# autonomousvision/LaRa

Hardware: AMD Instinct MI355X
Metric: novel-view frames/sec @512x512 (4-view in, 2DGS fwd+bwd) (higher is better)
Workload: dtype f32 raster + bf16-MFMA/f32-accumulate encoder (+ bf16-autocast coarse decoder MLP, as the reference's bf16-mixed)

## Files before the change

### lara_amd/csrc/abi.hip

```cpp
#include <stdlib.h>
#include <string.h>

#include "common.h"

static thread_local int g_last_hip_error = 0;
void l2d_set_hip_error(hipError_t e) { g_last_hip_error = (int)e; }

#include <atomic>
#include <mutex>
#include <map>
#include <utility>
#include <vector>
namespace {
struct ProfRec { const char *name; hipEvent_t a, b; };
std::atomic<bool> g_prof_on{false};
std::mutex g_prof_mu;
std::vector<ProfRec> g_prof_log;
std::vector<hipEvent_t> g_prof_pool;
hipEvent_t prof_event() {
    if (!g_prof_pool.empty()) { hipEvent_t e = g_prof_pool.back(); g_prof_pool.pop_back(); return e; }
    hipEvent_t e = nullptr;
    (void)hipEventCreate(&e);
    return e;
}
}

L2dProfScope::L2dProfScope(const char *name, hipStream_t stream) : slot(-1), s(stream) {
    if (!g_prof_on.load(std::memory_order_relaxed)) return;
    std::lock_guard<std::mutex> lk(g_prof_mu);
    ProfRec r{name, prof_event(), prof_event()};
    (void)hipEventRecord(r.a, s);
    g_prof_log.push_back(r);
    slot = (int)g_prof_log.size() - 1;
}
L2dProfScope::~L2dProfScope() {
    if (slot < 0) return;
    std::lock_guard<std::mutex> lk(g_prof_mu);
    if (slot < (int)g_prof_log.size()) (void)hipEventRecord(g_prof_log[slot].b, s);
}

namespace {

bool make_view(const lara2dgs_view *view, ViewDev &v) {
    if (!view) return false;
    if (view->P < 0 || view->image_height <= 0 || view->image_width <= 0) return false;
    if (view->sh_degree < 0 || view->sh_degree > 3) return false;
    if (view->capacity < 0 || view->capacity > 0xffffffffll) return false;
    if (!view->bg || !view->viewmatrix || !view->projmatrix || !view->campos) return false;
    v.P = view->P;
    v.deg = view->sh_degree;
    v.M = view->sh_coeffs;
    v.H = view->image_height;
    v.W = view->image_width;
    v.gx = (v.W + TILE - 1) / TILE;
    v.gy = (v.H + TILE - 1) / TILE;
    v.tiles = v.gx * v.gy;
    if (v.gx > 65535 || v.gy > 65535) return false;
    v.scale_modifier = view->scale_modifier;
// ... 396 lines not shown
```

### lara_amd/csrc/encoder_bwd.hip

```cpp
#include <cstdlib>

#include "mfma_gemm.h"
#include "mlp_fused.h"
#include "group_attn.h"
#include "../../include/lara_groupattn.h"

namespace {

struct TnP {
    const unsigned short *A, *B;
    float *part;
    const int *nbr;
    int M, lda, ldb, N, Kc, T, chunk, tiles;
};
constexpr int TN_GROUP_MAX = 6;
struct TnGroup {
    TnP p[TN_GROUP_MAX];
    int first_slot[TN_GROUP_MAX + 1];
    int count;
};

__device__ __forceinline__ bf16x8 pack_lo(const uint32_t *w) {
    union { uint32_t u[4]; bf16x8 v; } r;
#pragma unroll
    for (int d = 0; d < 4; d++) r.u[d] = __builtin_amdgcn_perm(w[2 * d + 1], w[2 * d], 0x05040100u);
    return r.v;
}
__device__ __forceinline__ bf16x8 pack_hi(const uint32_t *w) {
    union { uint32_t u[4]; bf16x8 v; } r;
#pragma unroll
    for (int d = 0; d < 4; d++) r.u[d] = __builtin_amdgcn_perm(w[2 * d + 1], w[2 * d], 0x07060302u);
    return r.v;
}
// ... 581 lines not shown
#pragma unroll
            for (int u = 0; u < 16; u++) v[u] = part[(size_t)(q + 16 * u) * stride + c];
#pragma unroll
            for (int u = 0; u < 8; u++) v[u] += v[u + 8];
#pragma unroll
            for (int u = 0; u < 4; u++) v[u] += v[u + 4];
            s += (v[0] + v[2]) + (v[1] + v[3]);
        }
        for (; q < parts; q += 16) s += part[(size_t)q * stride + c];
    }
    red[sl][lane] = s;
    __syncthreads();
    if (sl == 0 && c < n) {
        float t = red[0][lane];
        for (int k = 1; k < 16; k++) t += red[k][lane];
        g.dst[which][c] += t;
    }
}

__global__ void __launch_bounds__(256)
neighbour_table_kernel(int *__restrict__ nbr, const int M, const int R, const int zero_row, const int row_bytes) {
    const int m = blockIdx.x * 256 + threadIdx.x;
    if (m >= M) return;
    int b, d, h, w;
    token_to_voxel(m, R, b, d, h, w);
    for (int tap = 0; tap < 27; tap++) {
        const int nd = d + tap / 9 - 1, nh = h + (tap / 3) % 3 - 1, nw = w + tap % 3 - 1;
        const bool in = (unsigned)nd < (unsigned)R && (unsigned)nh < (unsigned)R && (unsigned)nw < (unsigned)R;
        nbr[(size_t)tap * M + m] = (in ? voxel_to_token(b, nd, nh, nw, R) : zero_row) * row_bytes;
    }
}

constexpr int LNB_ROWS = 128;
template <bool DY_BF16>
__global__ void __launch_bounds__(256)
ln_bwd_kernel(const void *dy_, const float *__restrict__ x, const float *__restrict__ gamma, const float eps,
              const float *skip, float *dx_out, unsigned short *__restrict__ dx_bf16, float *__restrict__ part,
              const int tokens) {
    const float *dy = (const float *)dy_;
    const unsigned short *dyh = (const unsigned short *)dy_;
    auto load_dy = [&](const size_t tok, const int lane) {
        if (DY_BF16) {
            const ushort4 h = ((const ushort4 *)(dyh + tok * 256))[lane];
            return make_float4(bf2f(h.x), bf2f(h.y), bf2f(h.z), bf2f(h.w));
        }
        return ((const float4 *)(dy + tok * 256))[lane];
    };
    __shared__ float red[4][12][64];
    const int wave = threadIdx.x >> 6, lane = threadIdx.x & 63;
    const float4 g = ((const float4 *)gamma)[lane];
    float pg[4] = {0.f, 0.f, 0.f, 0.f}, pb[4] = {0.f, 0.f, 0.f, 0.f}, po[4] = {0.f, 0.f, 0.f, 0.f};
    const int tok0 = blockIdx.x * LNB_ROWS + wave * (LNB_ROWS / 4);
    const int nrow = min(LNB_ROWS / 4, tokens - tok0);
    const float4 z4 = make_float4(0.f, 0.f, 0.f, 0.f);
    float4 vn = z4, dn = z4, kn = z4;
    if (nrow > 0) {
        vn = ((const float4 *)(x + (size_t)tok0 * 256))[lane];
        dn = load_dy((size_t)tok0, lane);
        if (skip) kn = ((const float4 *)(skip + (size_t)tok0 * 256))[lane];
    }
    for (int i = 0; i < nrow; i++) {
        const int tok = tok0 + i;
        const float4 v = vn, d = dn, k = kn;
        if (i + 1 < nrow) {
            vn = ((const float4 *)(x + (size_t)(tok + 1) * 256))[lane];
            dn = load_dy((size_t)(tok + 1), lane);
            if (skip) kn = ((const float4 *)(skip + (size_t)(tok + 1) * 256))[lane];
        }
        float s = v.x + v.y + v.z + v.w;
#pragma unroll
        for (int o = 32; o > 0; o >>= 1) s += __shfl_xor(s, o, 64);
        const float mean = s * (1.0f / 256.0f);
        const float c0 = v.x - mean, c1 = v.y - mean, c2 = v.z - mean, c3 = v.w - mean;
        float q = c0 * c0 + c1 * c1 + c2 * c2 + c3 * c3;
#pragma unroll
        for (int o = 32; o > 0; o >>= 1) q += __shfl_xor(q, o, 64);
        const float rstd = 1.0f / sqrtf(q * (1.0f / 256.0f) + eps);
        const float h0 = c0 * rstd, h1 = c1 * rstd, h2 = c2 * rstd, h3 = c3 * rstd;
        const float a0 = d.x * g.x, a1 = d.y * g.y, a2 = d.z * g.z, a3 = d.w * g.w;
        float sa = a0 + a1 + a2 + a3, sh = a0 * h0 + a1 * h1 + a2 * h2 + a3 * h3;
#pragma unroll
        for (int o = 32; o > 0; o >>= 1) { sa += __shfl_xor(sa, o, 64); sh += __shfl_xor(sh, o, 64); }
        sa *= (1.0f / 256.0f); sh *= (1.0f / 256.0f);
        const float4 r = make_float4(rstd * (a0 - sa - h0 * sh) + k.x, rstd * (a1 - sa - h1 * sh) + k.y,
                                     rstd * (a2 - sa - h2 * sh) + k.z, rstd * (a3 - sa - h3 * sh) + k.w);
        ((float4 *)(dx_out + (size_t)tok * 256))[lane] = r;
        if (dx_bf16) {
            ushort4 hb;
            hb.x = f2bf(r.x); hb.y = f2bf(r.y); hb.z = f2bf(r.z); hb.w = f2bf(r.w);
            ((ushort4 *)(dx_bf16 + (size_t)tok * 256))[lane] = hb;
        }
        pg[0] += d.x * h0; pg[1] += d.y * h1; pg[2] += d.z * h2; pg[3] += d.w * h3;
        pb[0] += d.x; pb[1] += d.y; pb[2] += d.z; pb[3] += d.w;
        po[0] += r.x; po[1] += r.y; po[2] += r.z; po[3] += r.w;
    }
#pragma unroll
    for (int c = 0; c < 4; c++) { red[wave][c][lane] = pg[c]; red[wave][4 + c][lane] = pb[c]; red[wave][8 + c][lane] = po[c]; }
    __syncthreads();
    if (wave == 0) {
#pragma unroll
        for (int k = 0; k < 12; k++) {
            const float t = (red[0][k][lane] + red[1][k][lane]) + (red[2][k][lane] + red[3][k][lane]);
            part[(size_t)blockIdx.x * 768 + (k >> 2) * 256 + 4 * lane + (k & 3)] = t;
        }
    }
}

__global__ void __launch_bounds__(256)
colsum_bf16_kernel(const unsigned short *__restrict__ src, float *__restrict__ part, const int rows, const int C) {
    const int r0 = blockIdx.x * 64, r1 = min(rows, r0 + 64);
    for (int c2 = threadIdx.x; c2 < C / 2; c2 += 256) {
        float s0 = 0.f, s1 = 0.f;
        for (int rr = r0; rr < r1; rr++) {
            const uint32_t w = *(const uint32_t *)(src + (size_t)rr * C + 2 * c2);
            s0 += __uint_as_float(w << 16);
            s1 += __uint_as_float(w & 0xffff0000u);
        }
        part[(size_t)blockIdx.x * C + 2 * c2] = s0;
        part[(size_t)blockIdx.x * C + 2 * c2 + 1] = s1;
    }
}

__global__ void __launch_bounds__(256)
// ... 100 lines not shown
    if (active) {
#pragma unroll
        for (int d = 0; d < 8; d++) {
            s_kv[gl][j2 * 512 + h2 * 16 + d0 + d] = f2bf(dk[d]);
            s_kv[gl][j2 * 512 + 256 + h2 * 16 + d0 + d] = f2bf(dvv[d]);
        }
    }
    __syncthreads();
    if (active) {
        uint4 *oq = (uint4 *)(dQ + (size_t)g * 8 * 256);
        unsigned short *ok = dKV + ((size_t)g * 4 + (t >> 6)) * lddkv + (t & 63) * 8;
        oq[t] = ((const uint4 *)s_dq[gl])[t]; oq[t + 128] = ((const uint4 *)s_dq[gl])[t + 128];
        *(uint4 *)ok = ((const uint4 *)s_kv[gl])[t]; *(uint4 *)(ok + 2 * (size_t)lddkv) = ((const uint4 *)s_kv[gl])[t + 128];
    }
}

constexpr size_t TN_PART_BYTES = 128ull << 20;

inline int cu_count() {
    static const int cus = [] {
        int dev = 0, v = 0;
        if (hipGetDevice(&dev) != hipSuccess || hipDeviceGetAttribute(&v, hipDeviceAttributeMultiprocessorCount, dev) != hipSuccess) v = 0;
        return v > 0 ? v : 256;
    }();
    return cus;
}

struct TnJob {
    const unsigned short *A; int lda, N;
    const unsigned short *B; int ldb, Kc;
    int M;
    float *dst;
};
int gemm_tn_group(const TnJob *jobs, int count, float *part, hipStream_t s);
inline bool tn_ring_shape(int M, int N, int Kc, int lda, int ldb, const float *dst) {
    return M >= 128 && !(M & 127) && !(N & 255) && !(Kc & 7) && !(lda & 7) && !(ldb & 7) && (size_t)(M + 1) * lda * 2 < (1ull << 32) &&
           (size_t)(M + 1) * ldb * 2 < (1ull << 32) && M < (1 << 24) && ldb < (1 << 23) && (((uintptr_t)dst) & 15) == 0;
}

int gemm_tn(const unsigned short *A, int lda, int N, const unsigned short *B, int ldb, int Kc, int T, const int *nbr,
            int M, float *dst, float *part, hipStream_t s) {
    if (M <= 0 || (nbr && M < 16) || (N & 1) || (Kc & 1) || (T > 1 && (Kc & 127))) return LARA2DGS_E_INVALID;
    if ((size_t)(M + 1) * lda * 2 >= (1ull << 32) || (size_t)(M + 1) * ldb * 2 >= (1ull << 32) || M >= (1 << 24) || ldb >= (1 << 23))
        return LARA2DGS_E_INVALID;
    const size_t out_bytes = (size_t)N * T * Kc * 4;
    const int n = N * T * Kc;
    if (!nbr && T == 1 && tn_ring_shape(M, N, Kc, lda, ldb, dst)) {
        const TnJob j{A, lda, N, B, ldb, Kc, M, dst};
        return gemm_tn_group(&j, 1, part, s);
    }
    if (nbr && N == 256 && Kc == 256 && (M & 127) == 0 && !(lda & 7) && !(ldb & 7) && (((uintptr_t)dst | (uintptr_t)part) & 15) == 0) {
        const int cus = cu_count();
        static const hipError_t attr = hipFuncSetAttribute((const void *)gemm_tn_ring_kernel<true>,
                                                           hipFuncAttributeMaxDynamicSharedMemorySize, TR_RING * TR_STAGE);
        L2D_HIP(attr);
        const int g128 = M / 128;
        int splits = max(1, min(min(cus / T, g128), (int)(TN_PART_BYTES / out_bytes)));
        const int chunk = ((g128 + splits - 1) / splits) * 128;
        splits = (M + chunk - 1) / chunk;
        TnRingGroup g{};
        TnRingP &q = g.p[0];
        q.A = A; q.B = B; q.part = part; q.nbr = nbr; q.M = M; q.lda = lda; q.ldb = ldb; q.T = T; q.ntile = q.ktile = 1; q.Kc = 256;
        q.chunk = chunk; q.splits = splits;
        g.count = 1; g.first_wg[0] = 0; g.first_wg[1] = T * splits;
        L2D_LAUNCH_IN_SCOPE(s, gemm_tn_ring_kernel<true>, dim3(T * splits), dim3(512), TR_RING * TR_STAGE, g);
        L2D_LAUNCH_IN_SCOPE(s, accum_partials4_kernel, dim3((n / 4 + 63) / 64), dim3(256), 0, dst, part, n, splits, (size_t)n);
        return LARA2DGS_OK;
    }
    const int tiles = ((N + 127) / 128) * ((Kc + 127) / 128) * T;
    const int want = 1024;
    int splits = max(1, min(want / tiles, (int)(TN_PART_BYTES / out_bytes)));
    splits = max(8, splits & ~7);
    while (splits > 8 && M / splits < 256) splits -= 8;
    const int chunk = (((M + splits - 1) / splits) + 63) & ~63;
    TnP p{};
    p.A = A; p.B = B; p.part = part; p.nbr = nbr; p.M = M; p.lda = lda; p.ldb = ldb; p.N = N; p.Kc = Kc; p.T = T;
    p.chunk = chunk; p.tiles = tiles;
    if ((size_t)splits * out_bytes > TN_PART_BYTES) return LARA2DGS_E_INVALID;
    const bool staged = !((M & 31) || (N & 7) || (Kc & 7) || (lda & 7) || (ldb & 7));
    if (staged) {
        TnGroup g{};
        g.p[0] = p; g.count = 1; g.first_slot[0] = 0; g.first_slot[1] = tiles * splits / 8;
        if (nbr) L2D_LAUNCH_IN_SCOPE(s, (gemm_bf16_tn_lds_kernel<true>), dim3(tiles * splits), dim3(256), 0, g);
        else L2D_LAUNCH_IN_SCOPE(s, (gemm_bf16_tn_lds_kernel<false>), dim3(tiles * splits), dim3(256), 0, g);
    } else {
        if (nbr) L2D_LAUNCH_IN_SCOPE(s, (gemm_bf16_tn_kernel<true>), dim3(tiles * splits), dim3(256), 0, p);
        else L2D_LAUNCH_IN_SCOPE(s, (gemm_bf16_tn_kernel<false>), dim3(tiles * splits), dim3(256), 0, p);
    }
    if ((n & 3) == 0 && (((uintptr_t)dst | (uintptr_t)part) & 15) == 0 && (n / 4 + 63) / 64 < 128 && splits >= 64)
        L2D_LAUNCH_IN_SCOPE(s, accum_partials4_wide_kernel, dim3((n / 4 + 63) / 64), dim3(1024), 0, dst, part, n, splits, (size_t)n);
    else if ((n & 3) == 0 && (((uintptr_t)dst | (uintptr_t)part) & 15) == 0)
        L2D_LAUNCH_IN_SCOPE(s, accum_partials4_kernel, dim3((n / 4 + 63) / 64), dim3(256), 0, dst, part, n, splits, (size_t)n);
    else
        L2D_LAUNCH_IN_SCOPE(s, accum_partials_kernel, dim3((n + 63) / 64), dim3(256), 0, dst, part, n, splits, (size_t)n);
    return LARA2DGS_OK;
}

int gemm_tn_group(const TnJob *jobs, int count, float *part, hipStream_t s) {
    bool ok = count >= 1 && count <= TN_GROUP_MAX;
    int tiles_all = 0;
    for (int k = 0; k < count && ok; k++) {
        const TnJob &j = jobs[k];
        ok = !((j.M & 31) || (j.N & 7) || (j.Kc & 7) || (j.lda & 7) || (j.ldb & 7)) && ((j.N * j.Kc) & 3) == 0 &&
             (size_t)(j.M + 1) * j.lda * 2 < (1ull << 32) && (size_t)(j.M + 1) * j.ldb * 2 < (1ull << 32) && j.M < (1 << 24) &&
             j.ldb < (1 << 23) && (((uintptr_t)j.dst) & 15) == 0;
        tiles_all += ((j.N + 127) / 128) * ((j.Kc + 127) / 128);
    }
    if (!ok) {
        for (int k = 0; k < count; k++) {
            L2D_TRY(gemm_tn(jobs[k].A, jobs[k].lda, jobs[k].N, jobs[k].B, jobs[k].ldb, jobs[k].Kc, 1, nullptr, jobs[k].M,
                                   jobs[k].dst, part, s));
        }
        return LARA2DGS_OK;
    }
    bool ringable = true;
    long units = 0;
    for (int k = 0; k < count; k++) {
        const TnJob &j = jobs[k];
        ringable = ringable && tn_ring_shape(j.M, j.N, j.Kc, j.lda, j.ldb, j.dst);
        units += (long)(j.N / 256) * ((j.Kc + 255) / 256) * (j.M / 128);
    }
    if (ringable) {
        static const hipError_t attr = hipFuncSetAttribute((const void *)gemm_tn_ring_kernel<false>,
                                                           hipFuncAttributeMaxDynamicSharedMemorySize, TR_RING * TR_STAGE);
        L2D_HIP(attr);
        const int cus = cu_count();
        TnRingGroup g{};
        AccGroup a{};
        g.count = a.count = count;
        for (int cg = (int)max(1l, (units + cus - 1) / cus);; cg++) {
            int wgs = 0, rwg = 0;
            size_t off_f = 0;
            for (int k = 0; k < count; k++) {
                const TnJob &j = jobs[k];
                const int tiles = (j.N / 256) * ((j.Kc + 255) / 256), n = j.N * j.Kc, splits = (j.M / 128 + cg - 1) / cg;
                TnRingP &q = g.p[k];
                q.A = j.A; q.B = j.B; q.part = part + off_f; q.nbr = nullptr; q.M = j.M; q.lda = j.lda; q.ldb = j.ldb; q.T = 1;
                q.ntile = j.N / 256; q.ktile = (j.Kc + 255) / 256; q.Kc = j.Kc; q.chunk = cg * 128; q.splits = splits;
                g.first_wg[k] = wgs;
                wgs += tiles * splits;
                a.dst[k] = j.dst; a.part[k] = part + off_f; a.n[k] = n; a.parts[k] = splits; a.first_wg[k] = rwg;
                rwg += (n / 4 + 63) / 64;
                off_f += (size_t)splits * n;
            }
            g.first_wg[count] = wgs;
            a.first_wg[count] = rwg;
            if (wgs <= cus && off_f * 4 <= TN_PART_BYTES) break;
            if (cg > (1 << 20)) return LARA2DGS_E_INVALID;
        }
        L2D_LAUNCH_IN_SCOPE(s, gemm_tn_ring_kernel<false>, dim3(g.first_wg[count]), dim3(512), TR_RING * TR_STAGE, g);
        L2D_LAUNCH_IN_SCOPE(s, accum_partials4_group_kernel, dim3(a.first_wg[count]), dim3(256), 0, a);
        return LARA2DGS_OK;
    }
    const int want = 1280;
    int base = max(8, (want / tiles_all) & ~7);
    TnGroup g{};
    AccGroup a{};
    g.count = a.count = count;
    size_t off_f = 0;
    for (;;) {
        off_f = 0;
        int slot = 0, wg = 0;
        for (int k = 0; k < count; k++) {
            const TnJob &j = jobs[k];
            int splits = base;
            while (splits > 8 && j.M / splits < 256) splits -= 8;
            const int tiles = ((j.N + 127) / 128) * ((j.Kc + 127) / 128), n = j.N * j.Kc;
            TnP &p = g.p[k];
            p.A = j.A; p.B = j.B; p.part = part + off_f; p.nbr = nullptr; p.M = j.M; p.lda = j.lda; p.ldb = j.ldb; p.N = j.N; p.Kc = j.Kc;
            p.T = 1; p.chunk = (((j.M + splits - 1) / splits) + 63) & ~63; p.tiles = tiles;
            g.first_slot[k] = slot;
            slot += tiles * splits / 8;
            a.dst[k] = j.dst; a.part[k] = part + off_f; a.n[k] = n; a.parts[k] = splits; a.first_wg[k] = wg;
            wg += (n / 4 + 63) / 64;
            off_f += (size_t)splits * n;
        }
        g.first_slot[count] = slot;
        a.first_wg[count] = wg;
        if (off_f * 4 <= TN_PART_BYTES || base == 8) break;
        base -= 8;
    }
    if (off_f * 4 > TN_PART_BYTES) return LARA2DGS_E_INVALID;
    L2D_LAUNCH_IN_SCOPE(s, (gemm_bf16_tn_lds_kernel<false>), dim3(g.first_slot[count] * 8), dim3(256), 0, g);
    L2D_LAUNCH_IN_SCOPE(s, accum_partials4_group_kernel, dim3(a.first_wg[count]), dim3(256), 0, a);
    return LARA2DGS_OK;
}

struct RedList {
    RedGroup g{};
    int wgs = 0;
    bool overflow = false;
    void add(float *dst, const float *part, int n, int parts, int stride) {
        if (!dst) return;
        if (g.count >= RED_GROUP_MAX) { overflow = true; return; }
        const int k = g.count++;
        g.dst[k] = dst; g.part[k] = part; g.n[k] = n; g.parts[k] = parts; g.stride[k] = stride; g.first_wg[k] = wgs;
        wgs += (n + 63) / 64;
        g.first_wg[g.count] = wgs;
    }
    int launch(hipStream_t s) {
        if (overflow) return LARA2DGS_E_INVALID;
        if (g.count) L2D_LAUNCH_IN_SCOPE(s, reduce_group_kernel, dim3(wgs), dim3(1024), 0, g);
        g.count = 0; wgs = 0;
        return LARA2DGS_OK;
    }
};

int ln_bwd(const void *dy, bool dy_bf16, const float *x, const float *gamma, float eps, const float *skip, float *dx,
           unsigned short *dx_bf16, float *dgamma, float *dbeta, float *part, int M, hipStream_t s, RedList *later = nullptr) {
    const int blocks = (M + LNB_ROWS - 1) / LNB_ROWS;
    if (dy_bf16) L2D_LAUNCH_IN_SCOPE(s, ln_bwd_kernel<true>, dim3(blocks), dim3(256), 0, dy, x, gamma, eps, skip, dx, dx_bf16, part, M);
    else L2D_LAUNCH_IN_SCOPE(s, ln_bwd_kernel<false>, dim3(blocks), dim3(256), 0, dy, x, gamma, eps, skip, dx, dx_bf16, part, M);
    if (later) {
        later->add(dgamma, part, 256, blocks, 768);
        later->add(dbeta, part + 256, 256, blocks, 768);
    } else {
        L2D_LAUNCH_IN_SCOPE(s, accum_ln_partials_kernel, dim3(4, 3), dim3(1024), 0, dgamma, dbeta, (float *)nullptr, part, blocks);
// ... 49 lines not shown
    w.gb3 = take(b256); w.gb2 = take(b256);
    w.lnpart4 = take(4 * ((size_t)(M + LNB_ROWS - 1) / LNB_ROWS) * 768 * 4);
    w.total = o;
    return w;
}

int block_forward_keep(int M, int cond_dim, const float *x_in, const unsigned short *cond_bf16,
                       const lara_groupblock_weights *w, char *save, hipStream_t s) {
    const SaveWs L = save_layout(M);
    const int G = M / 8, Mkv = G * 4;
    unsigned short *xn1 = (unsigned short *)(save + L.xn1), *q = (unsigned short *)(save + L.q), *kv = (unsigned short *)(save + L.kv);
    unsigned short *o = (unsigned short *)(save + L.o), *xn2 = (unsigned short *)(save + L.xn2), *z = (unsigned short *)(save + L.z);
    unsigned short *h = (unsigned short *)(save + L.h), *xn3 = (unsigned short *)(save + L.xn3);
    float *x1 = (float *)(save + L.x1), *x2 = (float *)(save + L.x2);
    {
        GemmP p{};
        p.A = cond_bf16; p.W = w->wkv; p.C = kv; p.M = Mkv; p.N = 512; p.K = cond_dim;
        L2D_HIP(launch_gemm_ring<0, 0>(p, s));
    }
    {
        unsigned short *wqp = (unsigned short *)(save + L.wpack), *wop = wqp + 65536;
        L2D_LAUNCH_IN_SCOPE(s, pack_weight_frag_kernel, dim3(64), dim3(256), 0, w->wq, wqp, w->wo, wop);
        L2D_LAUNCH_IN_SCOPE(s, group_attn_fused2_kernel<true>, dim3((G + 3) / 4), dim3(64), 0, x_in, w->ln1_w, w->ln1_b, w->eps, wqp, kv, wop,
                            x1, G, xn1, q, o);
    }
    {
        MlpP p{};
        p.x1 = x1; p.x2 = x2; p.ln2_w = w->ln2_w; p.ln2_b = w->ln2_b; p.b1 = w->b1; p.b2 = w->b2; p.ln3_w = w->ln3_w; p.ln3_b = w->ln3_b;
        p.w1 = w->w1; p.w2 = w->w2; p.xn3 = xn3; p.stats = (float2 *)(save + L.stats); p.xn2 = xn2; p.z = z; p.h = h; p.eps = w->eps; p.M = M;
        L2D_HIP(launch_mlp_fused<1>(p, s));
    }
    return LARA2DGS_OK;
}

bool block_weights_ok(const lara_groupblock_weights *w) {
    return w && w->ln1_w && w->ln1_b && w->wq && w->wkv && w->wo && w->ln2_w && w->ln2_b && w->w1 && w->b1 && w->w2 &&
           w->b2 && w->ln3_w && w->ln3_b && w->wconv;
}

}

extern "C" {

int64_t lara_groupblock_backward_workspace_bytes(int32_t scenes, int32_t R) {
    if (scenes < 0 || R < 4 || (R & 1)) return LARA2DGS_E_INVALID;
    return (int64_t)bwd_layout((int64_t)scenes * R * R * R).total;
}

int64_t lara_groupblock_save_bytes(int32_t scenes, int32_t R) {
    if (scenes < 0 || R < 4 || (R & 1)) return LARA2DGS_E_INVALID;
    return (int64_t)save_layout((int64_t)scenes * R * R * R).total;
}

int lara_groupblock_save_offsets(int32_t scenes, int32_t R, int64_t *offsets, int32_t n) {
    if (scenes < 0 || R < 4 || (R & 1) || !offsets || n != 11) return LARA2DGS_E_INVALID;
    const SaveWs L = save_layout((int64_t)scenes * R * R * R);
    const size_t at[11] = {L.xn1, L.q, L.kv, L.o, L.x1, L.xn2, L.z, L.h, L.x2, L.xn3, L.stats};
    for (int i = 0; i < 11; i++) offsets[i] = (int64_t)at[i];
    return LARA2DGS_OK;
}

int lara_groupblock_forward_train(int32_t scenes, int32_t R, int32_t cond_dim, const float *x_in, float *x_out,
                                  const uint16_t *cond_bf16, const lara_groupblock_weights *w, void *saved,
                                  void *stream) {
    if (scenes < 0 || R < 4 || (R & 1) || cond_dim <= 0 || (cond_dim % 32) != 0 || !block_weights_ok(w)) return LARA2DGS_E_INVALID;
    if (scenes == 0) return LARA2DGS_OK;
// ... 40 lines not shown
    const int M = (int)M64, G = M / 8, Mkv = G * 4;
    hipStream_t s = (hipStream_t)stream;
    const BwdWs L = bwd_layout(M);
    const SaveWs S = save_layout(M);
    char *ws = (char *)workspace;
    if (!saved) {
        L2D_PROF("gbb_recompute", s);
        L2D_TRY(block_forward_keep(M, cond_dim, x_in, cond_bf16, w, ws + L.save, s));
    }
    const char *sv = saved ? (const char *)saved : ws + L.save;
    const unsigned short *xn1 = (const unsigned short *)(sv + S.xn1), *q = (const unsigned short *)(sv + S.q);
    const unsigned short *kv = (const unsigned short *)(sv + S.kv), *o = (const unsigned short *)(sv + S.o);
    const unsigned short *xn2 = (const unsigned short *)(sv + S.xn2), *h = (const unsigned short *)(sv + S.h);
    const unsigned short *xn3 = (const unsigned short *)(sv + S.xn3);
    unsigned short *z = (unsigned short *)(sv + S.z);
    const float *x1 = (const float *)(sv + S.x1), *x2 = (const float *)(sv + S.x2);
    unsigned short *gb = (unsigned short *)(ws + L.gb);
    unsigned short *gb3 = (unsigned short *)(ws + L.gb3), *gb2 = (unsigned short *)(ws + L.gb2);
    unsigned short *dzb = (unsigned short *)(ws + L.dzb), *dq = (unsigned short *)(ws + L.dq);
    unsigned short *dkv = dkv_ext ? dkv_ext : (unsigned short *)(ws + L.dkv);
    const int ld_dkv = dkv_ext ? lddkv : 512;
    unsigned short *dob = (unsigned short *)(ws + L.dob);
    unsigned short *tmpb = (unsigned short *)(ws + L.tmpf);
    float *tnpart = (float *)(ws + L.tnpart);
    const size_t lnset = ((size_t)(M + LNB_ROWS - 1) / LNB_ROWS) * 768;
    float *lnp4 = (float *)(ws + L.lnpart4);
    RedList red;
    int *nbr = (int *)(ws + L.nbr);
    if (!chained) {
        L2D_HIP(hipMemsetAsync(gb + (size_t)M * 256, 0, 512, s));
        L2D_LAUNCH_IN_SCOPE(s, neighbour_table_kernel, dim3((M + 255) / 256), dim3(256), 0, nbr, M, R, M, 512);
        L2D_LAUNCH_IN_SCOPE(s, cast_bf16_kernel, dim3((unsigned)(((size_t)M * 64 + 255) / 256)), dim3(256), 0, g, gb, (size_t)M * 64);
    }
    {
        L2D_PROF("gbb_dw_conv", s);
        L2D_TRY(gemm_tn(gb, 256, 256, xn3, 256, 256, 27, nbr, M, dw->wconv, tnpart, s));
    }
    {
        L2D_PROF("gbb_dx_conv", s);
        GemmP p{};
        p.A = gb; p.W = wt->wconv_t; p.C = g; p.resid = g; p.M = M; p.N = 256; p.K = CONV_K;
        p.R = R; p.Cin = CONV_CIN; p.zero_off = (uint32_t)((size_t)M * 512);
        p.C2 = gb3; p.lnx = x2; p.stats = (const float2 *)(sv + S.stats); p.gamma = w->ln3_w; p.colsum = lnp4;
        L2D_HIP(launch_gemm_ring<1, 9>(p, s));
        const int tiles = (M + RT - 1) / RT;
        red.add(dw->ln3_w, lnp4, 256, tiles, 768);
        red.add(dw->ln3_b, lnp4 + 256, 256, tiles, 768);
        red.add(dw->b2, lnp4 + 512, 256, tiles, 768);
    }
    {
        L2D_PROF("gbb_dx_mlp", s);
        MlpP p{};
        p.gin = gb3; p.w1 = wt->w2_t; p.w2 = wt->w1_t; p.z = z; p.h = dzb; p.gout = tmpb; p.part_b1 = lnp4 + lnset; p.M = M;
        L2D_HIP(launch_mlp_fused<3>(p, s));
        red.add(dw->b1, lnp4 + lnset, 512, (M + 127) / 128, 512);
    }
    {
        L2D_PROF("gbb_ln_bwd", s);
        L2D_TRY(ln_bwd(tmpb, true, x1, w->ln2_w, w->eps, g, g, gb2, dw->ln2_w, dw->ln2_b, lnp4 + 2 * lnset, M, s, &red));
    }
    {
        L2D_PROF("gbb_dx_attn", s);
        L2D_TRY(gemm_nt<0>(gb2, wt->wo_t, dob, M, 256, 256, nullptr, s));
        L2D_LAUNCH_IN_SCOPE(s, group_attn_bwd_kernel, dim3((G + 1) / 2), dim3(256), 0, q, kv, dob, dq, dkv, G, ld_dkv);
        if (!dkv_ext) L2D_TRY(gemm_nt<1>(dkv, wt->wkv_t, dcond, Mkv, cond_dim, 512, dcond, s));
        L2D_TRY(gemm_nt<0>(dq, wt->wq_t, tmpb, M, 256, 256, nullptr, s));
    }
    {
        L2D_PROF("gbb_ln_bwd", s);
        L2D_TRY(ln_bwd(tmpb, true, x_in, w->ln1_w, w->eps, g, g, gb, dw->ln1_w, dw->ln1_b, lnp4 + 3 * lnset, M, s, &red));
        L2D_TRY(red.launch(s));
    }
    {
        L2D_PROF("gbb_dw_linear", s);
        const TnJob jobs[5] = {{gb3, 256, 256, h, 512, 512, M, dw->w2},
                               {dzb, 512, 512, xn2, 256, 256, M, dw->w1},
                               {gb2, 256, 256, o, 256, 256, M, dw->wo},
                               {dq, 256, 256, xn1, 256, 256, M, dw->wq},
                               {dkv, ld_dkv, 512, cond_bf16, cond_dim, cond_dim, Mkv, dw->wkv}};
        L2D_TRY(gemm_tn_group(jobs, 5, tnpart, s));
    }
    return LARA2DGS_OK;
}

int64_t lara_voltrans_head_backward_workspace_bytes(int32_t scenes, int32_t R, int32_t Cout) {
    if (scenes < 0 || R < 4 || (R & 1) || Cout <= 0 || (Cout & 15)) return LARA2DGS_E_INVALID;
    const size_t M = (size_t)scenes * R * R * R;
    return (int64_t)(up256(M * 512) + up256(M * 16 * Cout) + up256(M * 1024) + up256(((M + 63) / 64) * 4 * (size_t)max(768, 8 * Cout)) +
                     TN_PART_BYTES);
}

int lara_voltrans_head_backward(int32_t scenes, int32_t R, const float *x, const float *ln_w, const float *ln_b,
                                float eps, const uint16_t *wdeconv_t, int32_t Cout, const float *dout, float *g,
                                float *d_ln_w, float *d_ln_b, float *d_wdeconv, float *d_bias8, void *workspace,
                                void *stream) {
    if (scenes < 0 || R < 4 || (R & 1) || Cout <= 0 || (Cout & 15)) return LARA2DGS_E_INVALID;
    if (scenes == 0) return LARA2DGS_OK;
    if (!x || !ln_w || !ln_b || !wdeconv_t || !dout || !g || !d_ln_w || !d_ln_b || !d_wdeconv || !d_bias8 || !workspace)
        return LARA2DGS_E_INVALID;
    const int M = scenes * R * R * R, N8 = 8 * Cout;
    hipStream_t s = (hipStream_t)stream;
    char *ws = (char *)workspace;
    size_t off = 0;
    unsigned short *xn = (unsigned short *)(ws + off); off += up256((size_t)M * 512);
    unsigned short *dog = (unsigned short *)(ws + off); off += up256((size_t)M * 16 * Cout);
    float *tmpf = (float *)(ws + off); off += up256((size_t)M * 1024);
    float *lnpart = (float *)(ws + off); off += up256(((size_t)(M + 63) / 64) * 4 * (size_t)max(768, N8));
    float *tnpart = (float *)(ws + off);
    L2D_PROF("vtb_head", s);
    L2D_LAUNCH_IN_SCOPE(s, ln_cast_kernel, dim3((M + 3) / 4), dim3(256), 0, x, ln_w, ln_b, eps, xn, (float2 *)nullptr, M);
    {
        const size_t n = (size_t)M * 2 * Cout;
        L2D_LAUNCH_IN_SCOPE(s, deconv_grad_gather_kernel, dim3((unsigned)((n + 255) / 256)), dim3(256), 0, dout, dog, M, R, Cout);
    }
    L2D_TRY(colsum_bf16(dog, M, N8, d_bias8, lnpart, s));
    L2D_TRY(gemm_tn(dog, N8, N8, xn, 256, 256, 1, nullptr, M, d_wdeconv, tnpart, s));
    L2D_TRY(gemm_nt<0>(dog, wdeconv_t, tmpf, M, 256, N8, nullptr, s));
    L2D_TRY(ln_bwd(tmpf, true, x, ln_w, eps, nullptr, g, nullptr, d_ln_w, d_ln_b, lnpart, M, s));
    return LARA2DGS_OK;
}


int lara_gemm_nt_bf16(int32_t M, int32_t N, int32_t K, const uint16_t *A, const uint16_t *W, void *C, int32_t c_fp32,
                      void *stream) {
    if (M < 0 || N < 0 || K <= 0 || (K & 31)) return LARA2DGS_E_INVALID;
    if (M == 0 || N == 0) return LARA2DGS_OK;
    if (!A || !W || !C) return LARA2DGS_E_INVALID;
    if ((size_t)M * K * 2 >= (1ull << 32) || (size_t)N * K * 2 >= (1ull << 32)) return LARA2DGS_E_INVALID;
    GemmP p{};
    p.A = A; p.W = W; p.C = C; p.M = M; p.N = N; p.K = K;
    L2D_HIP(c_fp32 ? launch_gemm_ring<0, 8>(p, (hipStream_t)stream) : launch_gemm_ring<0, 0>(p, (hipStream_t)stream));
    return LARA2DGS_OK;
}

int lara_gemm_tn_bf16(int32_t M, int32_t N, int32_t Kc, const uint16_t *A, const uint16_t *B, float *dst,
                      void *workspace, void *stream) {
    if (M <= 0 || (M & 15) || N <= 0 || Kc <= 0 || !A || !B || !dst || !workspace) return LARA2DGS_E_INVALID;
    return gemm_tn(A, N, N, B, Kc, Kc, 1, nullptr, M, dst, (float *)workspace, (hipStream_t)stream);
}

int64_t lara_gemm_tn_workspace_bytes(void) { return (int64_t)TN_PART_BYTES; }

int lara_layernorm256_backward(int32_t rows, const float *dy, const float *x, const float *gamma, float eps,
                               const float *skip, float *dx, float *dgamma, float *dbeta, void *workspace,
                               void *stream) {
    if (rows <= 0 || !dy || !x || !gamma || !dx || !dgamma || !dbeta || !workspace) return LARA2DGS_E_INVALID;
    return ln_bwd(dy, false, x, gamma, eps, skip, dx, nullptr, dgamma, dbeta, (float *)workspace, rows, (hipStream_t)stream);
}

// ... 11 lines not shown
```

### lara_amd/csrc/launch.h

```cpp
#pragma once
#include <hip/hip_runtime.h>

#include "../../include/lara2dgs.h"

void l2d_set_hip_error(hipError_t e);
static inline int l2d_fail(hipError_t e) {
    l2d_set_hip_error(e);
    return LARA2DGS_E_LAUNCH;
}

struct L2dProfScope {
    int slot;
    hipStream_t s;
    L2dProfScope(const char *name, hipStream_t stream);
    ~L2dProfScope();
};
#define L2D_PROF(name, stream) L2dProfScope prof_scope__(name, stream)

#define L2D_HIP(...)                                        \
    do {                                                    \
        const hipError_t e__ = (__VA_ARGS__);               \
        if (e__ != hipSuccess) return l2d_fail(e__);        \
    } while (0)
#define L2D_FAIL_INTERNAL() return l2d_fail(hipSuccess)
#define L2D_TRY(...)                                        \
    do {                                                    \
        const int rc__ = (__VA_ARGS__);                     \
        if (rc__ != LARA2DGS_OK) return rc__;               \
    } while (0)

#define L2D_LAUNCH_ERR(stream, kernel, grid, block, lds, ...)                  \
    ({                                                                         \
        hipLaunchKernelGGL(kernel, grid, block, lds, stream, __VA_ARGS__);     \
        hipGetLastError();                                                     \
    })
#define L2D_LAUNCH_IN_SCOPE(stream, kernel, grid, block, lds, ...) L2D_HIP(L2D_LAUNCH_ERR(stream, kernel, grid, block, lds, __VA_ARGS__))
#define L2D_LAUNCH(label, stream, kernel, grid, block, lds, ...)               \
    do {                                                                       \
        {                                                                      \
            L2D_PROF(label, stream);                                           \
            hipLaunchKernelGGL(kernel, grid, block, lds, stream, __VA_ARGS__); \
        }                                                                      \
        L2D_HIP(hipGetLastError());                                            \
    } while (0)
```

Baseline: 981.0.

## Add optional side-stream overlap for weight-gradient GEMMs and tune LN backward

Adds an env-gated side stream that runs the conv and linear weight-gradient GEMMs (optionally split into pieces) concurrently with the main-stream data-gradient chain in the encoder block backward. The volume head backward also forks its colsum and deconv weight GEMM onto the side stream, using a separate partials buffer. The LayerNorm backward kernel switches to ds_swizzle/bpermute reductions, pointer-increment addressing and a waves-per-EU hint to cut reduction and address overhead. Overlap is off by default; when enabled it adds event synchronisation and competes for CUs with the main-stream work.

New measurement: 971.7. About the same (-0.9%).

```diff
diff --git a/lara_amd/csrc/abi.hip b/lara_amd/csrc/abi.hip
--- a/lara_amd/csrc/abi.hip
+++ b/lara_amd/csrc/abi.hip
@@ -24,6 +24,8 @@
     return e;
 }
 }
+
+bool l2d_profile_on() { return g_prof_on.load(std::memory_order_relaxed); }
 
 L2dProfScope::L2dProfScope(const char *name, hipStream_t stream) : slot(-1), s(stream) {
     if (!g_prof_on.load(std::memory_order_relaxed)) return;
diff --git a/lara_amd/csrc/encoder_bwd.hip b/lara_amd/csrc/encoder_bwd.hip
--- a/lara_amd/csrc/encoder_bwd.hip
+++ b/lara_amd/csrc/encoder_bwd.hip
@@ -1,4 +1,6 @@
 #include <cstdlib>
+#include <type_traits>
+#include <mutex>
 
 #include "mfma_gemm.h"
 #include "mlp_fused.h"
@@ -646,63 +648,72 @@
 }
 
 constexpr int LNB_ROWS = 128;
+template <int O>
+__device__ __forceinline__ float lnb_xor(const float v, const int idx32) {
+    if constexpr (O < 32) return __int_as_float(__builtin_amdgcn_ds_swizzle(__float_as_int(v), (O << 10) | 0x1f));
+    else return __int_as_float(__builtin_amdgcn_ds_bpermute(idx32, __float_as_int(v)));
+}
+__device__ __forceinline__ float lnb_sum(float s, const int idx32) {
+    s += lnb_xor<32>(s, idx32); s += lnb_xor<16>(s, idx32); s += lnb_xor<8>(s, idx32);
+    s += lnb_xor<4>(s, idx32); s += lnb_xor<2>(s, idx32); s += lnb_xor<1>(s, idx32);
+    return s;
+}
 template <bool DY_BF16>
-__global__ void __launch_bounds__(256)
+__global__ void __launch_bounds__(256) __attribute__((amdgpu_waves_per_eu(8, 8)))
 ln_bwd_kernel(const void *dy_, const float *__restrict__ x, const float *__restrict__ gamma, const float eps,
               const float *skip, float *dx_out, unsigned short *__restrict__ dx_bf16, float *__restrict__ part,
               const int tokens) {
-    const float *dy = (const float *)dy_;
-    const unsigned short *dyh = (const unsigned short *)dy_;
-    auto load_dy = [&](const size_t tok, const int lane) {
-        if (DY_BF16) {
-            const ushort4 h = ((const ushort4 *)(dyh + tok * 256))[lane];
-            return make_float4(bf2f(h.x), bf2f(h.y), bf2f(h.z), bf2f(h.w));
-        }
-        return ((const float4 *)(dy + tok * 256))[lane];
+    using DyRow = typename std::conditional<DY_BF16, ushort4, float4>::type;
+    auto widen = [](const DyRow w) {
+        if constexpr (DY_BF16) return make_float4(bf2f(w.x), bf2f(w.y), bf2f(w.z), bf2f(w.w));
+        else return w;
     };
     __shared__ float red[4][12][64];
-    const int wave = threadIdx.x >> 6, lane = threadIdx.x & 63;
+    const int wave = __builtin_amdgcn_readfirstlane(threadIdx.x >> 6), lane = threadIdx.x & 63;
+    const int idx32 = (lane ^ 32) << 2;
     const float4 g = ((const float4 *)gamma)[lane];
     float pg[4] = {0.f, 0.f, 0.f, 0.f}, pb[4] = {0.f, 0.f, 0.f, 0.f}, po[4] = {0.f, 0.f, 0.f, 0.f};
     const int tok0 = blockIdx.x * LNB_ROWS + wave * (LNB_ROWS / 4);
     const int nrow = min(LNB_ROWS / 4, tokens - tok0);
     const float4 z4 = make_float4(0.f, 0.f, 0.f, 0.f);
-    float4 vn = z4, dn = z4, kn = z4;
+    const float4 *xr = (const float4 *)(x + (size_t)tok0 * 256);
+    const DyRow *dr = (const DyRow *)dy_ + (size_t)tok0 * 64;
+    const float4 *kr = skip ? (const float4 *)(skip + (size_t)tok0 * 256) : nullptr;
+    float4 *orow = (float4 *)(dx_out + (size_t)tok0 * 256);
+    ushort4 *brow = (ushort4 *)(dx_bf16 + (size_t)tok0 * 256);
+    float4 vn = z4, kn = z4;
+    DyRow dn{};
     if (nrow > 0) {
-        vn = ((const float4 *)(x + (size_t)tok0 * 256))[lane];
-        dn = load_dy((size_t)tok0, lane);
-        if (skip) kn = ((const float4 *)(skip + (size_t)tok0 * 256))[lane];
+        vn = xr[lane];
+        dn = dr[lane];
+        if (skip) kn = kr[lane];
     }
     for (int i = 0; i < nrow; i++) {
-        const int tok = tok0 + i;
-        const float4 v = vn, d = dn, k = kn;
+        const float4 v = vn, d = widen(dn), k = kn;
         if (i + 1 < nrow) {
-            vn = ((const float4 *)(x + (size_t)(tok + 1) * 256))[lane];
-            dn = load_dy((size_t)(tok + 1), lane);
-            if (skip) kn = ((const float4 *)(skip + (size_t)(tok + 1) * 256))[lane];
-        }
-        float s = v.x + v.y + v.z + v.w;
-#pragma unroll
-        for (int o = 32; o > 0; o >>= 1) s += __shfl_xor(s, o, 64);
+            xr += 64; dr += 64; kr += 64;
+            vn = xr[lane];
+            dn = dr[lane];
+            if (skip) kn = kr[lane];
+        }
+        const float s = lnb_sum(v.x + v.y + v.z + v.w, idx32);
         const float mean = s * (1.0f / 256.0f);
         const float c0 = v.x - mean, c1 = v.y - mean, c2 = v.z - mean, c3 = v.w - mean;
-        float q = c0 * c0 + c1 * c1 + c2 * c2 + c3 * c3;
-#pragma unroll
-        for (int o = 32; o > 0; o >>= 1) q += __shfl_xor(q, o, 64);
+        const float q = lnb_sum(c0 * c0 + c1 * c1 + c2 * c2 + c3 * c3, idx32);
         const float rstd = 1.0f / sqrtf(q * (1.0f / 256.0f) + eps);
         const float h0 = c0 * rstd, h1 = c1 * rstd, h2 = c2 * rstd, h3 = c3 * rstd;
         const float a0 = d.x * g.x, a1 = d.y * g.y, a2 = d.z * g.z, a3 = d.w * g.w;
-        float sa = a0 + a1 + a2 + a3, sh = a0 * h0 + a1 * h1 + a2 * h2 + a3 * h3;
-#pragma unroll
-        for (int o = 32; o > 0; o >>= 1) { sa += __shfl_xor(sa, o, 64); sh += __shfl_xor(sh, o, 64); }
+        float sa = lnb_sum(a0 + a1 + a2 + a3, idx32), sh = lnb_sum(a0 * h0 + a1 * h1 + a2 * h2 + a3 * h3, idx32);
         sa *= (1.0f / 256.0f); sh *= (1.0f / 256.0f);
         const float4 r = make_float4(rstd * (a0 - sa - h0 * sh) + k.x, rstd * (a1 - sa - h1 * sh) + k.y,
                                      rstd * (a2 - sa - h2 * sh) + k.z, rstd * (a3 - sa - h3 * sh) + k.w);
-        ((float4 *)(dx_out + (size_t)tok * 256))[lane] = r;
+        orow[lane] = r;
+        orow += 64;
         if (dx_bf16) {
             ushort4 hb;
             hb.x = f2bf(r.x); hb.y = f2bf(r.y); hb.z = f2bf(r.z); hb.w = f2bf(r.w);
-            ((ushort4 *)(dx_bf16 + (size_t)tok * 256))[lane] = hb;
+            brow[lane] = hb;
+            brow += 64;
         }
         pg[0] += d.x * h0; pg[1] += d.y * h1; pg[2] += d.z * h2; pg[3] += d.w * h3;
         pb[0] += d.x; pb[1] += d.y; pb[2] += d.z; pb[3] += d.w;
@@ -869,7 +880,7 @@
     int M;
     float *dst;
 };
-int gemm_tn_group(const TnJob *jobs, int count, float *part, hipStream_t s);
+int gemm_tn_group(const TnJob *jobs, int count, float *part, hipStream_t s, int from = 0, int to = -1);
 inline bool tn_ring_shape(int M, int N, int Kc, int lda, int ldb, const float *dst) {
     return M >= 128 && !(M & 127) && !(N & 255) && !(Kc & 7) && !(lda & 7) && !(ldb & 7) && (size_t)(M + 1) * lda * 2 < (1ull << 32) &&
            (size_t)(M + 1) * ldb * 2 < (1ull << 32) && M < (1 << 24) && ldb < (1 << 23) && (((uintptr_t)dst) & 15) == 0;
@@ -933,7 +944,10 @@
     return LARA2DGS_OK;
 }
 
-int gemm_tn_group(const TnJob *jobs, int count, float *part, hipStream_t s) {
+int gemm_tn_group(const TnJob *jobs, int count, float *part, hipStream_t s, int from, int to) {
+    if (to < 0) to = count;
+    if (from < 0 || from >= to || to > count) return LARA2DGS_E_INVALID;
+    const int sub = to - from;
     bool ok = count >= 1 && count <= TN_GROUP_MAX;
     int tiles_all = 0;
     for (int k = 0; k < count && ok; k++) {
@@ -944,7 +958,7 @@
         tiles_all += ((j.N + 127) / 128) * ((j.Kc + 127) / 128);
     }
     if (!ok) {
-        for (int k = 0; k < count; k++) {
+        for (int k = from; k < to; k++) {
             L2D_TRY(gemm_tn(jobs[k].A, jobs[k].lda, jobs[k].N, jobs[k].B, jobs[k].ldb, jobs[k].Kc, 1, nullptr, jobs[k].M,
                                    jobs[k].dst, part, s));
         }
@@ -985,8 +999,18 @@
             if (wgs <= cus && off_f * 4 <= TN_PART_BYTES) break;
             if (cg > (1 << 20)) return LARA2DGS_E_INVALID;
         }
-        L2D_LAUNCH_IN_SCOPE(s, gemm_tn_ring_kernel<false>, dim3(g.first_wg[count]), dim3(512), TR_RING * TR_STAGE, g);
-        L2D_LAUNCH_IN_SCOPE(s, accum_partials4_group_kernel, dim3(a.first_wg[count]), dim3(256), 0, a);
+        if (sub < count) {
+            const int g0 = g.first_wg[from], a0 = a.first_wg[from];
+            for (int k = 0; k < sub; k++) {
+                g.p[k] = g.p[from + k]; g.first_wg[k] = g.first_wg[from + k] - g0;
+                a.dst[k] = a.dst[from + k]; a.part[k] = a.part[from + k]; a.n[k] = a.n[from + k]; a.parts[k] = a.parts[from + k];
+                a.first_wg[k] = a.first_wg[from + k] - a0;
+            }
+            g.first_wg[sub] = g.first_wg[to] - g0; a.first_wg[sub] = a.first_wg[to] - a0;
+            g.count = a.count = sub;
+        }
+        L2D_LAUNCH_IN_SCOPE(s, gemm_tn_ring_kernel<false>, dim3(g.first_wg[sub]), dim3(512), TR_RING * TR_STAGE, g);
+        L2D_LAUNCH_IN_SCOPE(s, accum_partials4_group_kernel, dim3(a.first_wg[sub]), dim3(256), 0, a);
         return LARA2DGS_OK;
     }
     const int want = 1280;
@@ -1018,8 +1042,18 @@
         base -= 8;
     }
     if (off_f * 4 > TN_PART_BYTES) return LARA2DGS_E_INVALID;
-    L2D_LAUNCH_IN_SCOPE(s, (gemm_bf16_tn_lds_kernel<false>), dim3(g.first_slot[count] * 8), dim3(256), 0, g);
-    L2D_LAUNCH_IN_SCOPE(s, accum_partials4_group_kernel, dim3(a.first_wg[count]), dim3(256), 0, a);
+    if (sub < count) {
+        const int s0 = g.first_slot[from], a0 = a.first_wg[from];
+        for (int k = 0; k < sub; k++) {
+            g.p[k] = g.p[from + k]; g.first_slot[k] = g.first_slot[from + k] - s0;
+            a.dst[k] = a.dst[from + k]; a.part[k] = a.part[from + k]; a.n[k] = a.n[from + k]; a.parts[k] = a.parts[from + k];
+            a.first_wg[k] = a.first_wg[from + k] - a0;
+        }
+        g.first_slot[sub] = g.first_slot[to] - s0; a.first_wg[sub] = a.first_wg[to] - a0;
+        g.count = a.count = sub;
+    }
+    L2D_LAUNCH_IN_SCOPE(s, (gemm_bf16_tn_lds_kernel<false>), dim3(g.first_slot[sub] * 8), dim3(256), 0, g);
+    L2D_LAUNCH_IN_SCOPE(s, accum_partials4_group_kernel, dim3(a.first_wg[sub]), dim3(256), 0, a);
     return LARA2DGS_OK;
 }
 
@@ -1135,6 +1169,70 @@
     }
     return LARA2DGS_OK;
 }
+
+constexpr int ENC_BWD_OVERLAP_DEFAULT = 0;
+int overlap_mode() {
+    static const int mode = [] {
+        const char *e = getenv("LARA_ENC_BWD_OVERLAP");
+        if (!e || !*e) return ENC_BWD_OVERLAP_DEFAULT;
+        const int v = atoi(e);
+        return v <= 0 ? 0 : (v >= 3 ? 3 : 1);
+    }();
+    return mode;
+}
+enum { EV_FORK, EV_MLP, EV_NORM2, EV_ATTN, EV_CONVDW, EV_JOIN, EV_COUNT };
+constexpr int SIDE_DEVICES_MAX = 64;
+struct SideLane {
+    std::mutex mu;
+    hipStream_t side = nullptr;
+    hipEvent_t ev[EV_COUNT] = {};
+};
+SideLane g_lanes[SIDE_DEVICES_MAX];
+
+struct SideRun {
+    SideLane *lane = nullptr;
+    hipStream_t main = nullptr, side = nullptr;
+    bool forked = false;
+    ~SideRun() {
+        if (!lane) return;
+        if (forked && hipEventRecord(lane->ev[EV_JOIN], side) == hipSuccess) (void)hipStreamWaitEvent(main, lane->ev[EV_JOIN], 0);
+        lane->mu.unlock();
+    }
+    bool on() const { return lane != nullptr; }
+    int begin(hipStream_t s) {
+        main = side = s;
+        if (!overlap_mode() || l2d_profile_on()) return LARA2DGS_OK;
+        int dev = 0;
+        L2D_HIP(hipGetDevice(&dev));
+        if (dev < 0 || dev >= SIDE_DEVICES_MAX) return LARA2DGS_OK;
+        SideLane *l = &g_lanes[dev];
+        l->mu.lock();
+        if (!l->side) {
+            int least = 0, greatest = 0;
+            hipStream_t st = nullptr;
+            hipError_t e = hipDeviceGetStreamPriorityRange(&least, &greatest);
+            if (e == hipSuccess) e = hipStreamCreateWithPriority(&st, hipStreamNonBlocking, least);
+            for (int k = 0; k < EV_COUNT && e == hipSuccess; k++) e = hipEventCreateWithFlags(&l->ev[k], hipEventDisableTiming);
+            if (e != hipSuccess) {
+                for (int k = 0; k < EV_COUNT; k++) if (l->ev[k]) { (void)hipEventDestroy(l->ev[k]); l->ev[k] = nullptr; }
+                if (st) (void)hipStreamDestroy(st);
+                l->mu.unlock();
+                return l2d_fail(e);
+            }
+            l->side = st;
+        }
+        lane = l;
+        side = l->side;
+        return LARA2DGS_OK;
+    }
+    int side_after_main(int ev) {
+        if (!lane) return LARA2DGS_OK;
+        L2D_HIP(hipEventRecord(lane->ev[ev], main));
+        L2D_HIP(hipStreamWaitEvent(side, lane->ev[ev], 0));
+        forked = true;
+        return LARA2DGS_OK;
+    }
+};
 
 bool block_weights_ok(const lara_groupblock_weights *w) {
     return w && w->ln1_w && w->ln1_b && w->wq && w->wkv && w->wo && w->ln2_w && w->ln2_b && w->w1 && w->b1 && w->w2 &&
@@ -1241,10 +1339,21 @@
         L2D_LAUNCH_IN_SCOPE(s, neighbour_table_kernel, dim3((M + 255) / 256), dim3(256), 0, nbr, M, R, M, 512);
         L2D_LAUNCH_IN_SCOPE(s, cast_bf16_kernel, dim3((unsigned)(((size_t)M * 64 + 255) / 256)), dim3(256), 0, g, gb, (size_t)M * 64);
     }
+    SideRun run;
+    L2D_TRY(run.begin(s));
+    hipStream_t sd = run.side;
+    const int pieces = run.on() && overlap_mode() == 3 ? 3 : 1;
+    const TnJob jobs[5] = {{gb3, 256, 256, h, 512, 512, M, dw->w2},
+                           {dzb, 512, 512, xn2, 256, 256, M, dw->w1},
+                           {gb2, 256, 256, o, 256, 256, M, dw->wo},
+                           {dq, 256, 256, xn1, 256, 256, M, dw->wq},
+                           {dkv, ld_dkv, 512, cond_bf16, cond_dim, cond_dim, Mkv, dw->wkv}};
+    L2D_TRY(run.side_after_main(EV_FORK));
     {
-        L2D_PROF("gbb_dw_conv", s);
-        L2D_TRY(gemm_tn(gb, 256, 256, xn3, 256, 256, 27, nbr, M, dw->wconv, tnpart, s));
-    }
+        L2D_PROF("gbb_dw_conv", sd);
+        L2D_TRY(gemm_tn(gb, 256, 256, xn3, 256, 256, 27, nbr, M, dw->wconv, tnpart, sd));
+    }
+    L2D_HIP(run.on() ? hipEventRecord(run.lane->ev[EV_CONVDW], sd) : hipSuccess);
     {
         L2D_PROF("gbb_dx_conv", s);
         GemmP p{};
@@ -1264,29 +1373,37 @@
         L2D_HIP(launch_mlp_fused<3>(p, s));
         red.add(dw->b1, lnp4 + lnset, 512, (M + 127) / 128, 512);
     }
+    if (pieces == 3) {
+        L2D_TRY(run.side_after_main(EV_MLP));
+        L2D_TRY(gemm_tn_group(jobs, 5, tnpart, sd, 0, 2));
+    }
     {
         L2D_PROF("gbb_ln_bwd", s);
         L2D_TRY(ln_bwd(tmpb, true, x1, w->ln2_w, w->eps, g, g, gb2, dw->ln2_w, dw->ln2_b, lnp4 + 2 * lnset, M, s, &red));
+    }
+    if (pieces == 3) {
+        L2D_TRY(run.side_after_main(EV_NORM2));
+        L2D_TRY(gemm_tn_group(jobs, 5, tnpart, sd, 2, 3));
     }
     {
         L2D_PROF("gbb_dx_attn", s);
         L2D_TRY(gemm_nt<0>(gb2, wt->wo_t, dob, M, 256, 256, nullptr, s));
         L2D_LAUNCH_IN_SCOPE(s, group_attn_bwd_kernel, dim3((G + 1) / 2), dim3(256), 0, q, kv, dob, dq, dkv, G, ld_dkv);
+        if (run.on()) {
+            L2D_TRY(run.side_after_main(EV_ATTN));
+            L2D_TRY(pieces == 3 ? gemm_tn_group(jobs, 5, tnpart, sd, 3, 5) : gemm_tn_group(jobs, 5, tnpart, sd));
+        }
         if (!dkv_ext) L2D_TRY(gemm_nt<1>(dkv, wt->wkv_t, dcond, Mkv, cond_dim, 512, dcond, s));
         L2D_TRY(gemm_nt<0>(dq, wt->wq_t, tmpb, M, 256, 256, nullptr, s));
     }
+    if (run.on()) L2D_HIP(hipStreamWaitEvent(s, run.lane->ev[EV_CONVDW], 0));
     {
         L2D_PROF("gbb_ln_bwd", s);
         L2D_TRY(ln_bwd(tmpb, true, x_in, w->ln1_w, w->eps, g, g, gb, dw->ln1_w, dw->ln1_b, lnp4 + 3 * lnset, M, s, &red));
         L2D_TRY(red.launch(s));
     }
-    {
+    if (!run.on()) {
         L2D_PROF("gbb_dw_linear", s);
-        const TnJob jobs[5] = {{gb3, 256, 256, h, 512, 512, M, dw->w2},
-                               {dzb, 512, 512, xn2, 256, 256, M, dw->w1},
-                               {gb2, 256, 256, o, 256, 256, M, dw->wo},
-                               {dq, 256, 256, xn1, 256, 256, M, dw->wq},
-                               {dkv, ld_dkv, 512, cond_bf16, cond_dim, cond_dim, Mkv, dw->wkv}};
         L2D_TRY(gemm_tn_group(jobs, 5, tnpart, s));
     }
     return LARA2DGS_OK;
@@ -1296,7 +1413,7 @@
     if (scenes < 0 || R < 4 || (R & 1) || Cout <= 0 || (Cout & 15)) return LARA2DGS_E_INVALID;
     const size_t M = (size_t)scenes * R * R * R;
     return (int64_t)(up256(M * 512) + up256(M * 16 * Cout) + up256(M * 1024) + up256(((M + 63) / 64) * 4 * (size_t)max(768, 8 * Cout)) +
-                     TN_PART_BYTES);
+                     TN_PART_BYTES + up256(((M + 63) / 64) * 4 * (size_t)(8 * Cout)));
 }
 
 int lara_voltrans_head_backward(int32_t scenes, int32_t R, const float *x, const float *ln_w, const float *ln_b,
@@ -1315,15 +1432,19 @@
     unsigned short *dog = (unsigned short *)(ws + off); off += up256((size_t)M * 16 * Cout);
     float *tmpf = (float *)(ws + off); off += up256((size_t)M * 1024);
     float *lnpart = (float *)(ws + off); off += up256(((size_t)(M + 63) / 64) * 4 * (size_t)max(768, N8));
-    float *tnpart = (float *)(ws + off);
+    float *tnpart = (float *)(ws + off); off += TN_PART_BYTES;
+    float *colpart = (float *)(ws + off);
     L2D_PROF("vtb_head", s);
     L2D_LAUNCH_IN_SCOPE(s, ln_cast_kernel, dim3((M + 3) / 4), dim3(256), 0, x, ln_w, ln_b, eps, xn, (float2 *)nullptr, M);
     {
         const size_t n = (size_t)M * 2 * Cout;
         L2D_LAUNCH_IN_SCOPE(s, deconv_grad_gather_kernel, dim3((unsigned)((n + 255) / 256)), dim3(256), 0, dout, dog, M, R, Cout);
     }
-    L2D_TRY(colsum_bf16(dog, M, N8, d_bias8, lnpart, s));
-    L2D_TRY(gemm_tn(dog, N8, N8, xn, 256, 256, 1, nullptr, M, d_wdeconv, tnpart, s));
+    SideRun run;
+    L2D_TRY(run.begin(s));
+    L2D_TRY(run.side_after_main(EV_FORK));
+    L2D_TRY(colsum_bf16(dog, M, N8, d_bias8, colpart, run.side));
+    L2D_TRY(gemm_tn(dog, N8, N8, xn, 256, 256, 1, nullptr, M, d_wdeconv, tnpart, run.side));
     L2D_TRY(gemm_nt<0>(dog, wdeconv_t, tmpf, M, 256, N8, nullptr, s));
     L2D_TRY(ln_bwd(tmpf, true, x, ln_w, eps, nullptr, g, nullptr, d_ln_w, d_ln_b, lnpart, M, s));
     return LARA2DGS_OK;
diff --git a/lara_amd/csrc/launch.h b/lara_amd/csrc/launch.h
--- a/lara_amd/csrc/launch.h
+++ b/lara_amd/csrc/launch.h
@@ -15,6 +15,7 @@
     L2dProfScope(const char *name, hipStream_t stream);
     ~L2dProfScope();
 };
+bool l2d_profile_on();
 #define L2D_PROF(name, stream) L2dProfScope prof_scope__(name, stream)
 
 #define L2D_HIP(...)                                        \
```
